# nmonette/TO-UED

Hardware: AMD Instinct MI355X
Metric: agent-env-steps/sec (inner rollout) at num_agents=512; meta-updates/sec (higher is better)
Workload: dtype f32; 1 GPU; C2 LPG meta-gradient env_mode=tabular num_agents=512 num_mini_batches=1 W=64 T=20 K=5 score_function=random; num_agents=512, agents_per_gpu=512, env_workers=64, train_rollout_len=20, num_agent_updates=5, parallelism=dp1 (agent axis)

## Files before the change

to-ued_amd/csrc/gru.hip:

```cpp
#include <stdlib.h>
#include <string.h>
#include <algorithm>
#include "common.h"

extern "C" size_t toued_wgrad_workspace_floats(int ra, int rb, long K);
extern "C" int toued_wgrad(int ra, int rb, long K, const float* A, long lda, const float* B, long ldb, float* C,
                           float* work, size_t work_floats, hipStream_t stream);
extern "C" int toued_wgrad_ldc(int ra, int rb, long K, const float* A, long lda, const float* B, long ldb, float* C,
                               int ldc, float* work, size_t work_floats, hipStream_t stream);
extern "C" size_t toued_rowsum_workspace_floats(int ra, long K);
extern "C" int toued_rowsum_into(int ra, long K, const float* A, long lda, float* C, int ldc, float* work,
                                 size_t work_floats, hipStream_t stream);

typedef float floatx16 __attribute__((ext_vector_type(16)));
typedef float floatx4 __attribute__((ext_vector_type(4)));

#define HU 256
#define RB 32
#define LDH 33
#define NAUG 8
#define KQF 33
#define NTILE_F 32

struct EtaOff {
// ... 748 lines not shown
        const f16x4 h0 = *reinterpret_cast<const f16x4*>(&hB[0][ho]);
        const f16x4 h1 = *reinterpret_cast<const f16x4*>(&hB[1][ho]);
        const bf16x4 hr = *reinterpret_cast<const bf16x4*>(&hB[2][ho]);
        const unsigned sq = quad_soff(cbase + r0, h, g4);
        float sv[3][4];
        float us[3][4];
#pragma unroll
        for (int g = 0; g < 3; ++g) {
          const float4 v = *reinterpret_cast<const float4*>(&usc[g * HU + ub + 8 * g4]);
          us[g][0] = v.x; us[g][1] = v.y; us[g][2] = v.z; us[g][3] = v.w;
        }
        f16x4 n0, n1;
        bf16x4 nr;
#pragma unroll
        for (int e = 0; e < 4; ++e) {
          const int q = 4 * g4 + e;
          const float rg = sigm_r(acc[0][h][q] * us[0][e]);
          const float zg = sigm_r(acc[1][h][q] * us[1][e]);
          const float hn = acc[2][h][q] * us[2][e];
          const float ng = gate_n(ain[h][q], rg, hn);
          const float hin = (((float)h0[e] + (float)h1[e]) + (float)hr[e]) * (1.0f / HSCALE);
          const float hh = (1.0f - zg) * ng + zg * hin;
          split_carry(dn ? 0.0f : hh, n0, n1, nr, e);
          sv[0][e] = rg;
          sv[1][e] = zg;
          sv[2][e] = hn;
          if (SAVE) st_u(rs_hin, vslab, slab_soff(cbase + r0, h, qunit(q)), hin);
          const float rl = fmaxf(hh, 0.0f);
          const float4 w0 = whl[qunit(q) * 3], w1 = whl[qunit(q) * 3 + 1], w2 = whl[qunit(q) * 3 + 2];
          hp_loc[0] += rl * w0.x; hp_loc[1] += rl * w0.y; hp_loc[2] += rl * w0.z;
          hp_loc[3] += rl * w0.w; hp_loc[4] += rl * w1.x; hp_loc[5] += rl * w1.y;
          hp_loc[6] += rl * w1.z; hp_loc[7] += rl * w1.w; hp_loc[8] += rl * w2.x;
        }
        if (SAVE) {
          st4(rs_r, vq, sq, sv[0]);
          st4(rs_z, vq, sq, sv[1]);
          st4(rs_hn, vq, sq, sv[2]);
        }
        *reinterpret_cast<f16x4*>(&hB[0][ho]) = n0;
        *reinterpret_cast<f16x4*>(&hB[1][ho]) = n1;
        *reinterpret_cast<bf16x4*>(&hB[2][ho]) = nr;
      }
#pragma unroll
      for (int oo = 0; oo < 9; ++oo) {
        const float o = __shfl_xor(hp_loc[oo], 32);
        if (hi == 0) hp[(s & 1) * 4608 + (wave * 9 + oo) * 64 + row] = hp_loc[oo] + o;
      }
      GM_STAMP(1 + h);
    }
    FWD_STAMP(3);
    lds_barrier();
    FWD_STAMP(4);
    FWD_STAMP(5);
  }
  if (wave == 0) head_out(T - 1);
}

struct BwdArgs {
  int R, T, W, K;
  const uint8_t* done; long done_stride_k;
  const float4* A;
  const void* A6;
  const float* eta; EtaOff o;
  const float* y_hat; const float* d_pi_hat; const float* d_y_hat;
  const float* s_hin; const float* s_r; const float* s_z; const float* s_n; const float* s_hn;
  long M;
  float* DG;
  float* RH;
  float* DH;
  float* dX3; float* dX4;
  int8_t* CE;
  int F;
  float* SP;
  int stagger, stagger_mode;
  int wg_base;
};
#define SP_C (16 * HU)
#define SP_FLOATS (SP_C + 9 * 64)

template <int NT>
__global__ void __launch_bounds__(512, NT == 1 ? 4 : 1) k_gru_bwd(BwdArgs p) {
  constexpr int RBT = RB * NT;
  constexpr int LDT = RBT + 1;
  __shared__ float dgT[2 * HU * LDT];
  __shared__ float wi34[2 * 3 * HU];
  __shared__ float hv[9 * RBT];
  __shared__ float dxp[NGRP * 2 * RBT];
  const int tid = threadIdx.x, lane = tid & 63, wave = tid >> 6, hi = lane >> 5, col = lane & 31;
  const int nb = p.R / RBT;
  const int k = blockIdx.x / nb;
  const int r0 = (blockIdx.x - k * nb) * RBT;
  const int R = p.R, T = p.T, W = p.W;
  int a_[NT], w_[NT];
#pragma unroll
  for (int h = 0; h < NT; ++h) {
    const int row = r0 + RB * h + col;
    a_[h] = (r0 + RB * h) / W;
    w_[h] = row - a_[h] * W;
  }
  for (int i = tid; i < 2 * 3 * HU; i += 512) {
    const int f = 3 + i / (3 * HU), g = (i / HU) % 3, u = i % HU;
    const int base = g == 0 ? p.o.ir_w : g == 1 ? p.o.iz_w : p.o.in_w;
    wi34[i] = f < p.F ? p.eta[base + f * HU + u] : 0.0f;
  }
  float dh[NT][16];
#pragma unroll
  for (int h = 0; h < NT; ++h)
#pragma unroll
    for (int q = 0; q < 16; ++q) dh[h][q] = 0.0f;
  float wA[5];
#pragma unroll
  for (int kk = 0; kk < 5; ++kk) {
    const int o = 2 * kk + hi, u = 32 * wave + col;
    wA[kk] = o < 9 ? (o == 0 ? p.eta[p.o.pi_w + u] : p.eta[p.o.y_w + u * 8 + (o - 1)]) : 0.0f;
  }
  const uint8_t* done = p.done + (long)k * p.done_stride_k;
  const float4* Ab = p.A + lane;
  const __amdgpu_buffer_rsrc_t rs_hin = rsrc_of(p.s_hin), rs_r = rsrc_of(p.s_r), rs_z = rsrc_of(p.s_z),
                               rs_n = rsrc_of(p.s_n), rs_hn = rsrc_of(p.s_hn), rs_rh = rsrc_of(p.RH);
  const __amdgpu_buffer_rsrc_t rs_dg[4] = {rsrc_of(p.DG), rsrc_of(p.DG + 1L * HU * p.M),
                                           rsrc_of(p.DG + 2L * HU * p.M), rsrc_of(p.DG + 3L * HU * p.M)};
  __syncthreads();
  for (int t = 0; t < T; ++t) {
    const long ctr = ((long)k * T + t) * R;
    if (tid < RBT) {
      const long o = ctr + r0 + tid;
      float yh[8], dy[8], s = 0.0f;
      for (int j = 0; j < 8; ++j) {
        yh[j] = p.y_hat[((long)k * T * 8 + (long)t * 8 + j) * R + r0 + tid];
        dy[j] = p.d_y_hat[((long)k * T * 8 + (long)t * 8 + j) * R + r0 + tid];
        s += yh[j] * dy[j];
      }
      const float dpi = p.d_pi_hat[o];
      hv[tid] = dpi;
      p.DH[o] = dpi;
      for (int j = 0; j < 8; ++j) {
        const float v = yh[j] * (dy[j] - s);
        hv[(j + 1) * RBT + tid] = v;
        p.DH[(long)(j + 1) * p.M + o] = v;
      }
    }
    __syncthreads();
    float dhn_r[NT][16];
    const float* wil = wi34 + 32 * wave + 4 * hi;
#pragma unroll
    for (int h = 0; h < NT; ++h) {
      floatx16 hacc;
#pragma unroll
      for (int q = 0; q < 16; ++q) hacc[q] = 0.0f;
#pragma unroll
      for (int kk = 0; kk < 5; ++kk) {
        const int o = 2 * kk + hi;
        hacc = mfma32(wA[kk], o < 9 ? hv[o * RBT + RB * h + col] : 0.0f, hacc);
      }
      const unsigned vq = (unsigned)((((long)(32 * wave + 4 * hi + (col & 3))) * p.M + r0 + RB * h + (col & 28)) * 4);
      float dx3 = 0.0f, dx4 = 0.0f;
#pragma unroll
      for (int g4 = 0; g4 < 4; ++g4) {
        const unsigned so = (unsigned)(((long)8 * g4 * p.M + ctr) * 4);
        float v_hin[4], v_r[4], v_z[4], v_n[4], v_hn[4];
        ld4(rs_hin, vq, so, v_hin);
        ld4(rs_r, vq, so, v_r);
        ld4(rs_z, vq, so, v_z);
        ld4(rs_n, vq, so, v_n);
        ld4(rs_hn, vq, so, v_hn);
        quad_transpose(v_hin, lane);
        quad_transpose(v_r, lane);
        quad_transpose(v_z, lane);
        quad_transpose(v_n, lane);
        quad_transpose(v_hn, lane);
        float* o_rh = v_hin; float* o_dr = v_r; float* o_dz = v_z; float* o_dhn = v_n; float* o_dn = v_hn;
#pragma unroll
        for (int j = 0; j < 4; ++j) {
          const int q = 4 * g4 + j;
          const float hin = v_hin[j], rg = v_r[j], zg = v_z[j], ng = v_n[j], hn = v_hn[j];
          const float hout = (1.0f - zg) * ng + zg * hin;
          const float d = dh[h][q] + (hout > 0.0f ? hacc[q] : 0.0f);
          const float dn_ = d * (1.0f - zg);
          const float dz = d * (hin - ng);
          const float dnp = dn_ * (1.0f - ng * ng);
          const float dhn = dnp * rg;
          const float drp = dnp * hn * rg * (1.0f - rg);
          const float dzp = dz * zg * (1.0f - zg);
          dh[h][q] = d * zg;
          const int lo = (32 * wave + 4 * hi + qunit(q)) * LDT + RB * h + col;
          dgT[lo] = drp;
          dgT[HU * LDT + lo] = dzp;
          dhn_r[h][q] = dhn;
          o_rh[j] = fmaxf(hout, 0.0f); o_dr[j] = drp; o_dz[j] = dzp; o_dhn[j] = dhn; o_dn[j] = dnp;
          const int qu = qunit(q);
          dx3 += drp * wil[0 * HU + qu] + dzp * wil[1 * HU + qu] + dnp * wil[2 * HU + qu];
          dx4 += drp * wil[3 * HU + qu] + dzp * wil[4 * HU + qu] + dnp * wil[5 * HU + qu];
        }
        {
          const unsigned vb = (unsigned)(((long)(32 * wave + 4 * hi) * p.M + r0 + RB * h + col) * 4);
#pragma unroll
          for (int j = 0; j < 4; ++j) {
            const unsigned so1 = (unsigned)(((long)qunit(4 * g4 + j) * p.M + ctr) * 4);
            st_u(rs_rh, vb, so1, o_rh[j]);
            st_u(rs_dg[3], vb, so1, o_dn[j]);
          }
        }
      }
      dxp[((2 * wave + hi) * 2 + 0) * RBT + RB * h + col] = dx3;
      dxp[((2 * wave + hi) * 2 + 1) * RBT + RB * h + col] = dx4;
    }
    floatx16 acc[NT];
#pragma unroll
    for (int h = 0; h < NT; ++h)
#pragma unroll
      for (int q = 0; q < 16; ++q) acc[h][q] = 0.0f;
#pragma unroll 1
    for (int g = 0; g < 3; ++g) {
      if (g == 2) {
        __syncthreads();
#pragma unroll
        for (int h = 0; h < NT; ++h) {
          float* dgl = dgT + (32 * wave + 4 * hi) * LDT + RB * h + col;
#pragma unroll
          for (int q = 0; q < 16; ++q) dgl[qunit(q) * LDT] = dhn_r[h][q];
        }
      }
      if (g != 1) __syncthreads();
      if (g == 0) {
        store_gate_lds<NT>(dgT, rs_dg[0], p.M, ctr + r0, wave, lane);
        store_gate_lds<NT>(dgT + HU * LDT, rs_dg[1], p.M, ctr + r0, wave, lane);
      } else if (g == 2) {
        store_gate_lds<NT>(dgT, rs_dg[2], p.M, ctr + r0, wave, lane);
      }
      const float* dgs = dgT + (g == 1 ? HU * LDT : 0);
      float4 an = Ab[((wave * 3 + g) * 32 + 0) * 64];
#pragma unroll 2
      for (int kq = 0; kq < 32; ++kq) {
        const float4 av = an;
        if (kq + 1 < 32) an = Ab[((wave * 3 + g) * 32 + kq + 1) * 64];
#pragma unroll
        for (int e = 0; e < 4; ++e) {
          const float x = e == 0 ? av.x : e == 1 ? av.y : e == 2 ? av.z : av.w;
#pragma unroll
          for (int h = 0; h < NT; ++h) {
            const float b = dgs[(2 * (4 * kq + e) + hi) * LDT + RB * h + col];
            acc[h] = mfma32(x, b, acc[h]);
          }
        }
      }
    }
    __syncthreads();
    if (tid < RBT) {
      float s3 = 0.0f, s4 = 0.0f;
      for (int gq = 0; gq < NGRP; ++gq) { s3 += dxp[(gq * 2 + 0) * RBT + tid]; s4 += dxp[(gq * 2 + 1) * RBT + tid]; }
      p.dX3[ctr + r0 + tid] = s3;
      p.dX4[ctr + r0 + tid] = s4;
    }
#pragma unroll
    for (int h = 0; h < NT; ++h) {
      const bool dn = done[((size_t)a_[h] * T + t) * W + w_[h]] != 0;
#pragma unroll
      for (int q = 0; q < 16; ++q) dh[h][q] = dn ? 0.0f : dh[h][q] + acc[h][q];
    }
    __syncthreads();
  }
}


#ifdef BWD_STAMPS
__device__ unsigned long long g_bwd_stamps[64 * 32 * 8];
#define BWD_STAMP(ph)                                                                                  \
  do {                                                                                                 \
    if (blockIdx.x < 64 && tid == 0 && t < 32)                                                         \
      g_bwd_stamps[(blockIdx.x * 32 + t) * 8 + (ph)] = __builtin_amdgcn_s_memtime();                   \
  } while (0)
#define BWD_NWS 8
__device__ unsigned long long g_bwd_wstamps[64 * 32 * 8 * BWD_NWS];
__device__ int g_bwd_wsimd[64 * 8];
#define BWD_WSTAMP(ph)                                                                                 \
  do {                                                                                                 \
    if (blockIdx.x < 64 && lane_now() == 0 && t < 32)                                                  \
      g_bwd_wstamps[((blockIdx.x * 32 + t) * 8 + wave) * BWD_NWS + (ph)] = __builtin_amdgcn_s_memtime(); \
  } while (0)
#else
#define BWD_STAMP(ph) do {} while (0)
#define BWD_WSTAMP(ph) do {} while (0)
#endif

#ifndef BWD_PK
#define BWD_PK 1
#endif
template <bool SMALL>
__global__ void __launch_bounds__(512, 1) k_gru_bwd6n(BwdArgs p) {
  constexpr int RBT = 2 * RB;
  constexpr int PP = HU + 8;
  __shared__ __attribute__((aligned(16))) __bf16 dgB[3][RBT * PP];
  __shared__ float wi34[2 * 3 * HU];
  __shared__ float hv[9 * RBT];
  __shared__ __attribute__((aligned(8))) float dxp[8 * RBT * 2];
  __shared__ __attribute__((aligned(16))) float wsc[HU];
  __shared__ float rmx[8 * RBT];
  __shared__ float wIs[8 * 4 * 64];
  __shared__ float wAs[8 * 5 * 64];
  __shared__ int dns[RBT];
  __shared__ __attribute__((aligned(16))) float Atab[SMALL ? 32 * 64 : 4];
  __shared__ float hvs[SMALL ? 9 * RBT : 1];
  __shared__ floatx4 accl[SMALL ? 8 * 2 * 64 : 1];
  constexpr int DRP = HU + 4;
  static_assert(RBT * DRP * 4 <= 2 * RBT * PP * 2, "dr staging exceeds image slots 1-2");
  float* drs = reinterpret_cast<float*>(&dgB[1][0]);
  const int tid = threadIdx.x, lane = tid & 63, hi = lane >> 5, col = lane & 31;
  const int wave = __builtin_amdgcn_readfirstlane(tid >> 6);
  const int nb = p.R / RBT;
  const int bid = blockIdx.x + p.wg_base;
  const int k = bid / nb;
  const int r0 = (bid - k * nb) * RBT;
  const int R = p.R, T = p.T, W = p.W;
#ifdef BWD_STAMPS
  if (blockIdx.x < 64 && (tid & 63) == 0)
    g_bwd_wsimd[blockIdx.x * 8 + wave] = __builtin_amdgcn_s_getreg((1 << 11) | (4 << 6) | 4);
#endif
  for (int i = tid; i < 2 * 3 * HU; i += 512) {
    const int f = BWD_PK ? 3 + (i & 1) : 3 + i / (3 * HU), g = BWD_PK ? (i >> 1) / HU : (i / HU) % 3,
              u = BWD_PK ? (i >> 1) % HU : i % HU;
    const int base = g == 0 ? p.o.ir_w : g == 1 ? p.o.iz_w : p.o.in_w;
    wi34[i] = f < p.F ? p.eta[base + f * HU + u] : 0.0f;
  }
  for (int i = tid; i < HU; i += 512) wsc[i] = reinterpret_cast<const float*>(p.A6)[B6_SCALES + i];
  const int F = p.F;
  {
    float wI[4];
    load_win_frags(wI, p.eta, p.o, F, wave, lane);
#pragma unroll
    for (int kk = 0; kk < 4; ++kk) wIs[(wave * 4 + kk) * 64 + lane] = wI[kk];
  }
#pragma unroll
  for (int kk = 0; kk < 5; ++kk) {
    const int o = 2 * kk + hi, u = 32 * wave + col;
    wAs[(wave * 5 + kk) * 64 + lane] = o < 9 ? (o == 0 ? p.eta[p.o.pi_w + u] : p.eta[p.o.y_w + u * 8 + (o - 1)]) : 0.0f;
  }
  float dh[2][16];
#pragma unroll
  for (int h = 0; h < 2; ++h)
#pragma unroll
    for (int q = 0; q < 16; ++q) dh[h][q] = 0.0f;
  if (SMALL) {
    for (int i = tid; i < 9 * RBT; i += 512) hvs[i] = 0.0f;
    for (int i = tid; i < 8 * 2 * 64; i += 512) accl[i] = floatx4{0.0f, 0.0f, 0.0f, 0.0f};
  }
  constexpr bool st_rh = !SMALL, st_dn = !SMALL;
  const __amdgpu_buffer_rsrc_t rs_hin = rsrc_of(p.s_hin), rs_r = rsrc_of(p.s_r), rs_z = rsrc_of(p.s_z),
                               rs_hn = rsrc_of(p.s_hn), rs_rh = rsrc_of(SMALL ? p.s_hin : p.RH);
  const __amdgpu_buffer_rsrc_t rs_x = rsrc_of(p.s_hin + (size_t)HU * p.M);
  const __amdgpu_buffer_rsrc_t rs_dg[4] = {rsrc_of(p.DG), rsrc_of(p.DG + 1L * HU * p.M),
                                           rsrc_of(p.DG + 2L * HU * p.M),
                                           rsrc_of(SMALL ? p.DG : p.DG + 3L * HU * p.M)};
  constexpr bool st_DH = !SMALL;
  const __amdgpu_buffer_rsrc_t rs_yh = rsrc_of(p.y_hat), rs_dyh = rsrc_of(p.d_y_hat), rs_dpi = rsrc_of(p.d_pi_hat),
                               rs_DH = rsrc_of(SMALL ? p.dX3 : p.DH), rs_dx3 = rsrc_of(p.dX3), rs_dx4 = rsrc_of(p.dX4),
                               rs_done = rsrc_of(reinterpret_cast<const float*>(p.done + (long)k * p.done_stride_k));
  auto head_cot = [&](int t) {
    if (tid < RBT) {
      const int tl = lane_now();
      const unsigned vrw = (unsigned)tl * 4;
      int dnv;
      {
        const int rw = r0 + tl, a = rw / W;
        dnv = __builtin_amdgcn_raw_buffer_load_b8(rs_done, (a * T + t) * W + rw - a * W, 0, 0);
      }
      const long o = ((long)k * T + t) * R + r0;
      float yh[8], dy[8], s = 0.0f;
#pragma unroll
      for (int j = 0; j < 8; ++j) {
        const unsigned so = (unsigned)((((long)k * T * 8 + (long)t * 8 + j) * R + r0) * 4);
        yh[j] = ld_u(rs_yh, vrw, so);
        dy[j] = ld_u(rs_dyh, vrw, so);
      }
#pragma unroll
      for (int j = 0; j < 8; ++j) s += yh[j] * dy[j];
      const float dpi = ld_u(rs_dpi, vrw, (unsigned)(o * 4));
      float xr[6];
      if (SMALL) {
#pragma unroll
        for (int f = 0; f < 6; ++f)
          xr[f] = ld_u(rs_x, vrw, (unsigned)(((long)(f < F ? f : 0) * p.M + o) * 4));
      }
      dns[tl] = dnv;
      hv[tl] = dpi;
      if (st_DH) st_u(rs_DH, vrw, (unsigned)(o * 4), dpi);
      float hvv[9];
      hvv[0] = dpi;
#pragma unroll
      for (int j = 0; j < 8; ++j) {
        const float v = yh[j] * (dy[j] - s);
        hv[(j + 1) * RBT + tl] = v;
        hvv[j + 1] = v;
        if (st_DH) st_u(rs_DH, vrw, (unsigned)(((long)(j + 1) * p.M + o) * 4), v);
      }
      if (SMALL) {
        float* at = Atab + (tl >> 1) * 64 + 16 * (tl & 1);
#pragma unroll
        for (int c = 0; c < 4; ++c) {
          if (c >= 2) *reinterpret_cast<float4*>(at + 4 * c) = make_float4(0.0f, 0.0f, 0.0f, 0.0f);
          *reinterpret_cast<float4*>(at + 32 + 4 * c) = make_float4(0.0f, 0.0f, 0.0f, 0.0f);
        }
        at[6] = 0.0f;
        at[7] = 0.0f;
        *reinterpret_cast<float4*>(at) = make_float4(0 < F ? xr[0] : 0.0f, 1 < F ? xr[1] : 0.0f, 2 < F ? xr[2] : 0.0f,
                                                     3 < F ? xr[3] : 0.0f);
        *reinterpret_cast<float2*>(at + 4) = make_float2(4 < F ? xr[4] : 0.0f, 5 < F ? xr[5] : 0.0f);
        at[F] = 1.0f;
#pragma unroll
        for (int o9 = 0; o9 < 9; ++o9) at[32 + F + 1 + o9] = hvv[o9];
#pragma unroll
        for (int o9 = 0; o9 < 9; ++o9) hvs[o9 * RBT + tl] += hvv[o9];
      }
    }
  };
  const __amdgpu_buffer_rsrc_t rs_A = rsrc_of(reinterpret_cast<const float*>(p.A6));
  const unsigned vA = (unsigned)lane * 16;
  floatx16 acc[2];
  auto ldAh = [&](int ks, int g, int q) {
    const u32x4 x = __builtin_amdgcn_raw_buffer_load_b128(rs_A, (int)vA,
                                                          (int)((((ks * 8 + wave) * 3 + g) * 3 + q) * 1024), 0);
    return __builtin_bit_cast(f16x8, x);
  };
#ifndef BWD_RD
#define BWD_RD 4
#endif
  auto dg_vbyte = [&](int ub_, int col_) {
    return SMALL ? (unsigned)(ub_ * 128 + col_ * 4) : (unsigned)(((long)ub_ * p.M + r0 + col_) * 4);
  };
  auto dg_soff = [&](long ctr_, int uq, int h) {
    return SMALL ? (unsigned)((((ctr_ + r0) >> 5) + h) * 32768L + uq * 128)
                 : (unsigned)((((long)uq * p.M + ctr_) * 4) + 128 * h);
  };
  auto contract_h = [&](int g) {
    constexpr int RD = BWD_RD;
    f16x8 ring[RD][2], B[2][2];
    int sb = 0, sb1 = 1;
#pragma unroll
    for (int i = 0; i < RD; ++i)
#pragma unroll
      for (int q = 0; q < 2; ++q) ring[i][q] = ldAh(i, g, q);
    const int ln = lane_now(), bl = (ln & 31) * PP + 8 * (ln >> 5);
    auto ldB = [&](int ks, int h) {
#pragma unroll
      for (int q = 0; q < 2; ++q) B[h][q] = *reinterpret_cast<const f16x8*>(&dgB[q ? sb1 : sb][bl + RB * h * PP + 16 * ks]);
    };
    ldB(0, 0);
    ldB(0, 1);
    auto kstep = [&](int ks, f16x8 (&Ar)[2], bool reload) {
#pragma unroll
      for (int h = 0; h < 2; ++h) {
        acc[h] = mfma3h(Ar, B[h], acc[h]);
        if (ks + 1 < 16) ldB(ks + 1, h);
      }
      if (reload) {
#pragma unroll
        for (int q = 0; q < 2; ++q) Ar[q] = ldAh(ks + RD, g, q);
      }
      __builtin_amdgcn_sched_barrier(0);
    };
    constexpr int NG = (16 - RD) / RD;
#pragma nounroll
    for (int gi = 0; gi < NG; ++gi) {
#pragma unroll
      for (int j = 0; j < RD; ++j) kstep(gi * RD + j, ring[j], true);
    }
#pragma unroll
    for (int ks = NG * RD; ks < 16; ++ks) {
      kstep(ks, ring[ks % RD], ks + RD < 16);
      if (ks == 16 - RD) __builtin_amdgcn_sched_barrier(0);
      if (ks >= 12) __builtin_amdgcn_sched_barrier(0);
    }
  };
  auto put4h = [&](int row, int u0, const float (&v)[4], float sc) {
    f16x4 x0, x1;
#pragma unroll
    for (int e = 0; e < 4; ++e) split2h(v[e] * sc, x0, x1, e);
    *reinterpret_cast<f16x4*>(&dgB[0][row * PP + u0]) = x0;
    *reinterpret_cast<f16x4*>(&dgB[1][row * PP + u0]) = x1;
  };
  float* priv = reinterpret_cast<float*>(&dgB[0][0]) + 1056 * wave;
  auto small_mfma = [&](int h, int g4, const float (&dnq)[4], const float (&rhq)[4]) {
    const int ln = lane_now(), row = ln & 31, c = 2 * (g4 & 1) + (ln >> 5);
    const int wo = row * 16 + ((c ^ ((row >> 2) & 3)) << 2);
    *reinterpret_cast<float4*>(priv + wo) = make_float4(dnq[0], dnq[1], dnq[2], dnq[3]);
    *reinterpret_cast<float4*>(priv + 544 + wo) = make_float4(rhq[0], rhq[1], rhq[2], rhq[3]);
    if (g4 & 1) {
      const int l2 = lane_now(), kk = l2 >> 4, j = l2 & 15;
      const int rb = (kk >> 1) * 544 + (kk & 1) * 16 + (j & 3);
      floatx4& al = accl[(wave * 2 + (g4 >> 1)) * 64 + l2];
      floatx4 acc = al;
#pragma unroll
      for (int s2 = 0; s2 < 16; ++s2) {
        const float b = priv[rb + 32 * s2 + ((((j >> 2) ^ ((s2 >> 1) & 3))) << 2)];
        const float a = Atab[(16 * h + s2) * 64 + l2];
        acc = __builtin_amdgcn_mfma_f32_16x16x4f32(a, b, acc, 0, 0, 0);
      }
      al = acc;
    }
  };
#ifndef BWD_NR
#define BWD_NR 3
#endif
  constexpr int NR = BWD_NR;
  const int ub = 32 * wave + 4 * hi;
  float vr[NR][4][4];
  auto load_q = [&](long ctr_, int h, int g4, float (&v)[4][4]) {
    const unsigned vq = quad_vbyte(ub, col), sq = quad_soff(ctr_ + r0, h, g4);
    ld4(rs_hin, slab_vbyte(ub + (col & 3), col & 28), slab_soff(ctr_ + r0, h, 8 * g4), v[0]);
    ld4(rs_r, vq, sq, v[1]);
    ld4(rs_z, vq, sq, v[2]);
    ld4(rs_hn, vq, sq, v[3]);
  };
  float xa[4], xb[4];
  auto load_x = [&](long ctr_, int h, float (&x)[4]) {
#pragma unroll
    for (int kk = 0; kk < 4; ++kk) {
      const int ln = lane_now(), k = 2 * kk + (ln >> 5);
      x[kk] = ld_u(rs_x, (unsigned)((((long)(k < F ? k : 0)) * p.M + RB * h + (ln & 31)) * 4), (unsigned)((ctr_ + r0) * 4));
    }
  };
  auto load_first = [&](long ctr_) {
    load_x(ctr_, 0, xa);
#pragma unroll
    for (int qi = 0; qi < NR - 1; ++qi) load_q(ctr_, qi >> 2, qi & 3, vr[qi]);
  };
  if (p.stagger > 0 && blockIdx.x < 256) {
    const int ph = p.stagger_mode == 0 ? (blockIdx.x >> 3) & 1 : p.stagger_mode == 1 ? blockIdx.x & 1 : (blockIdx.x >> 3) & 3;
    for (int i = 0; i < ph * p.stagger; ++i) __builtin_amdgcn_s_sleep(127);
  }
  const long ctr0 = (long)k * T * R;
  for (int t = 0; t < T; ++t) {
    const long ctr = ctr0 + (long)t * R;
    BWD_STAMP(0);
    head_cot(t);
    lds_barrier();
    BWD_STAMP(1);
    BWD_WSTAMP(0);
    float dz_r[2][16], dhn_r[2][16];
    auto ubn = [&] { return 32 * wave + 4 * (lane_now() >> 5); };
    auto rown = [&](int h) { return RB * h + (lane_now() & 31); };
    auto st_q = [&](__amdgpu_buffer_rsrc_t rs, int h, int g4, const float (&v)[4]) {
#pragma unroll
      for (int e = 0; e < 4; ++e)
        st_u(rs, (unsigned)(((long)ub * p.M + r0 + RB * h + col) * 4),
             (unsigned)(((long)qunit(4 * g4 + e) * p.M + ctr) * 4), v[e]);
    };
    load_first(ctr);
    floatx16 ain;
    floatx16 hacc;
    float dx3 = 0.0f, dx4 = 0.0f;
    float rmr[2] = {0.0f, 0.0f};
#pragma unroll
    for (int qi = 0; qi < 8; ++qi) {
      const int h = qi >> 2, g4 = qi & 3;
      float (&v)[4][4] = vr[qi % NR];
      if (qi + NR - 1 < 8) load_q(ctr, (qi + NR - 1) >> 2, (qi + NR - 1) & 3, vr[(qi + NR - 1) % NR]);
      if (qi == 3) load_x(ctr, 1, xb);
      __builtin_amdgcn_sched_barrier(0);
      if (g4 == 0) {
#pragma unroll
        for (int q = 0; q < 16; ++q) hacc[q] = 0.0f;
#pragma unroll
        for (int kk = 0; kk < 5; ++kk) {
          const int ln = lane_now(), o = 2 * kk + (ln >> 5);
          hacc = mfma32(wAs[(wave * 5 + kk) * 64 + ln], o < 9 ? hv[o * RBT + RB * h + (ln & 31)] : 0.0f, hacc);
        }
        float wI[4];
#pragma unroll
        for (int kk = 0; kk < 4; ++kk) wI[kk] = wIs[(wave * 4 + kk) * 64 + lane];
        ain = gate_ain(wI, F, hi, [&](int k) { return h ? xb[k >> 1] : xa[k >> 1]; });
        dx3 = 0.0f;
        dx4 = 0.0f;
      }
      quad_transpose(v[0], lane);
      const float* wil = wi34 + ubn();
      float drq[4], rhq[4], dnq[4];
      if (BWD_PK) {
        const f2v* wil2 = reinterpret_cast<const f2v*>(wi34) + ubn();
        f2v dx34 = {dx3, dx4};
#pragma unroll
        for (int pp = 0; pp < 2; ++pp) {
          const int j0 = 2 * pp, q0 = 4 * g4 + j0;
          const f2v hin = {v[0][j0], v[0][j0 + 1]}, rg = {v[1][j0], v[1][j0 + 1]}, zg = {v[2][j0], v[2][j0 + 1]},
                    hn = {v[3][j0], v[3][j0 + 1]};
          const f2v ng = {gate_n(ain[q0], rg.x, hn.x), gate_n(ain[q0 + 1], rg.y, hn.y)};
          const f2v omz = 1.0f - zg;
          const f2v hout = omz * ng + zg * hin;
          const f2v hac = {hout.x > 0.0f ? hacc[q0] : 0.0f, hout.y > 0.0f ? hacc[q0 + 1] : 0.0f};
          const f2v d = f2v{dh[h][q0], dh[h][q0 + 1]} + hac;
          const f2v dn_ = d * omz;
          const f2v dz = d * (hin - ng);
          const f2v dnp = dn_ * (1.0f - ng * ng);
          const f2v dhn = dnp * rg;
          const f2v drp = dnp * hn * rg * (1.0f - rg);
          const f2v dzp = dz * zg * omz;
          const f2v dhv = d * zg;
#pragma unroll
          for (int e = 0; e < 2; ++e) {
            const int q = q0 + e, qu = qunit(q);
            dh[h][q] = dhv[e];
            drq[j0 + e] = drp[e];
            dz_r[h][q] = dzp[e];
            dhn_r[h][q] = dhn[e];
            rhq[j0 + e] = fmaxf(hout[e], 0.0f);
            dnq[j0 + e] = dnp[e];
            dx34 += f2v{drp[e], drp[e]} * wil2[0 * HU + qu] + f2v{dzp[e], dzp[e]} * wil2[1 * HU + qu] +
                    f2v{dnp[e], dnp[e]} * wil2[2 * HU + qu];
          }
        }
        dx3 = dx34.x;
        dx4 = dx34.y;
      }
#pragma unroll
      for (int jj = 0; jj < (BWD_PK ? 0 : 4); ++jj) {
        const int q = 4 * g4 + jj;
        const float hin = v[0][jj], rg = v[1][jj], zg = v[2][jj], hn = v[3][jj];
        const float ng = gate_n(ain[q], rg, hn);
        const float hout = (1.0f - zg) * ng + zg * hin;
        const float d = dh[h][q] + (hout > 0.0f ? hacc[q] : 0.0f);
        const float dn_ = d * (1.0f - zg);
        const float dz = d * (hin - ng);
        const float dnp = dn_ * (1.0f - ng * ng);
        const float dhn = dnp * rg;
        const float drp = dnp * hn * rg * (1.0f - rg);
        const float dzp = dz * zg * (1.0f - zg);
        dh[h][q] = d * zg;
        drq[jj] = drp;
        dz_r[h][q] = dzp;
        dhn_r[h][q] = dhn;
        const int qu = qunit(q);
        dx3 += drp * wil[0 * HU + qu] + dzp * wil[1 * HU + qu] + dnp * wil[2 * HU + qu];
        dx4 += drp * wil[3 * HU + qu] + dzp * wil[4 * HU + qu] + dnp * wil[5 * HU + qu];
        rhq[jj] = fmaxf(hout, 0.0f);
        dnq[jj] = dnp;
      }
      if (st_rh) st_q(rs_rh, h, g4, rhq);
      if (st_dn) st_q(rs_dg[3], h, g4, dnq);
      if (SMALL) small_mfma(h, g4, dnq, rhq);
      *reinterpret_cast<float4*>(&drs[rown(h) * DRP + ubn() + 8 * g4]) = make_float4(drq[0], drq[1], drq[2], drq[3]);
#pragma unroll
      for (int jj = 0; jj < 4; ++jj) rmr[h] = fmaxf(rmr[h], fabsf(drq[jj]));
      if (g4 == 3) {
        const float f3 = dx3 + __shfl_xor(dx3, 32), f4 = dx4 + __shfl_xor(dx4, 32);
        const int ln = lane_now();
        if (ln < 32) *reinterpret_cast<float2*>(dxp + (wave * RBT + RB * h + ln) * 2) = make_float2(f3, f4);
      }
      __builtin_amdgcn_sched_barrier(0);
    }
    BWD_STAMP(2);
    BWD_WSTAMP(1);
#pragma unroll
    for (int h = 0; h < 2; ++h) {
      float m = rmr[h];
#pragma unroll
      for (int q = 0; q < 16; ++q) m = fmaxf(m, fmaxf(fabsf(dz_r[h][q]), fabsf(dhn_r[h][q])));
      m = fmaxf(m, __shfl_xor(m, 32));
      const int ln = lane_now();
      if (ln < 32) rmx[wave * RBT + RB * h + ln] = m;
    }
    lds_barrier();
    BWD_STAMP(3);
    float bs[2];
#pragma unroll
    for (int h = 0; h < 2; ++h) {
      float m = 0.0f;
      const int cl = lane_now() & 31;
#pragma unroll
      for (int w8 = 0; w8 < 8; ++w8) m = fmaxf(m, rmx[w8 * RBT + RB * h + cl]);
      int sc = 0, ce = 127;
      if (m > 0.0f && m <= 3.0e38f) {
        int e;
        frexpf(m, &e);
        sc = min(40, max(-40, 14 - e));
        ce = min(126, max(-126, 14 - e));
      }
      bs[h] = ldexpf(1.0f, sc);
      if (p.CE && wave == 0 && lane_now() < 32) p.CE[ctr + r0 + rown(h)] = (int8_t)ce;
    }
    auto store_dg = [&](int g, int row, int g4, const float (&v)[4]) {
#pragma unroll
      for (int e = 0; e < 4; ++e)
        st_u(rs_dg[g], dg_vbyte(ub, col), dg_soff(ctr, qunit(4 * g4 + e), row >= RB ? 1 : 0), v[e]);
    };
    {
      f16x4 x1h[2][4];
#pragma unroll
      for (int h = 0; h < 2; ++h)
#pragma unroll
        for (int g4 = 0; g4 < 4; ++g4) {
          const int row = rown(h), un = ubn();
          const float4 v = *reinterpret_cast<const float4*>(&drs[row * DRP + un + 8 * g4]);
          const float v4[4] = {v.x, v.y, v.z, v.w};
          f16x4 x0;
#pragma unroll
          for (int e = 0; e < 4; ++e) split2h(v4[e] * bs[h], x0, x1h[h][g4], e);
          *reinterpret_cast<f16x4*>(&dgB[0][row * PP + un + 8 * g4]) = x0;
          store_dg(0, RB * h, g4, v4);
        }
      lds_barrier();
#pragma unroll
      for (int h = 0; h < 2; ++h)
#pragma unroll
        for (int g4 = 0; g4 < 4; ++g4)
          *reinterpret_cast<f16x4*>(&dgB[1][rown(h) * PP + ubn() + 8 * g4]) = x1h[h][g4];
      lds_barrier();
    }
    const int un0 = ubn();
#pragma unroll
    for (int g4 = 0; g4 < 4; ++g4) {
      const float4 w4 = *reinterpret_cast<const float4*>(&wsc[un0 + 8 * g4]);
      const float wv[4] = {w4.x, w4.y, w4.z, w4.w};
#pragma unroll
      for (int h = 0; h < 2; ++h)
#pragma unroll
        for (int e = 0; e < 4; ++e) acc[h][4 * g4 + e] = dh[h][4 * g4 + e] * (wv[e] * bs[h]);
    }
    BWD_STAMP(4);
    BWD_WSTAMP(2);
    contract_h(0);
    BWD_WSTAMP(3);
    lds_barrier();
    BWD_WSTAMP(4);
#pragma unroll
    for (int h = 0; h < 2; ++h)
#pragma unroll
      for (int g4 = 0; g4 < 4; ++g4) {
        const float v4[4] = {dz_r[h][4 * g4], dz_r[h][4 * g4 + 1], dz_r[h][4 * g4 + 2], dz_r[h][4 * g4 + 3]};
        put4h(rown(h), ubn() + 8 * g4, v4, bs[h]);
        store_dg(1, RB * h, g4, v4);
      }
    lds_barrier();
    BWD_STAMP(5);
    BWD_WSTAMP(5);
    contract_h(1);
    BWD_WSTAMP(6);
    lds_barrier();
    BWD_WSTAMP(7);
#pragma unroll
    for (int h = 0; h < 2; ++h)
#pragma unroll
      for (int g4 = 0; g4 < 4; ++g4) {
        const float v4[4] = {dhn_r[h][4 * g4], dhn_r[h][4 * g4 + 1], dhn_r[h][4 * g4 + 2], dhn_r[h][4 * g4 + 3]};
        put4h(rown(h), ubn() + 8 * g4, v4, bs[h]);
        store_dg(2, RB * h, g4, v4);
      }
    lds_barrier();
    BWD_STAMP(6);
    contract_h(2);
#pragma unroll
    for (int g4 = 0; g4 < 4; ++g4) {
      const float4 w4 = *reinterpret_cast<const float4*>(&wsc[32 * wave + 4 * (lane_now() >> 5) + 8 * g4]);
      const float wv[4] = {w4.x, w4.y, w4.z, w4.w};
#pragma unroll
      for (int h = 0; h < 2; ++h)
#pragma unroll
        for (int e = 0; e < 4; ++e) acc[h][4 * g4 + e] *= inv_pow2(wv[e] * bs[h]);
    }
    if (tid < RBT) {
      const int tl = lane_now();
      float s3 = 0.0f, s4 = 0.0f;
#pragma unroll
      for (int w8 = 0; w8 < 8; ++w8) {
        const float2 v = *reinterpret_cast<const float2*>(dxp + (w8 * RBT + tl) * 2);
        s3 += v.x;
        s4 += v.y;
      }
      st_u(rs_dx3, (unsigned)tl * 4, (unsigned)((ctr + r0) * 4), s3);
      st_u(rs_dx4, (unsigned)tl * 4, (unsigned)((ctr + r0) * 4), s4);
    }
#pragma unroll
    for (int h = 0; h < 2; ++h) {
      const bool dn = dns[RB * h + (lane_now() & 31)] != 0;
#pragma unroll
      for (int q = 0; q < 16; ++q) dh[h][q] = dn ? 0.0f : acc[h][q];
    }
    BWD_STAMP(7);
    lds_barrier();
  }
  if (SMALL) {
    float* out = p.SP + (size_t)bid * SP_FLOATS;
    const int ln = lane_now();
#pragma unroll
    for (int uh = 0; uh < 2; ++uh) {
      const floatx4 a = accl[(wave * 2 + uh) * 64 + ln];
#pragma unroll
      for (int r = 0; r < 4; ++r) out[(4 * (ln >> 4) + r) * HU + 32 * wave + 16 * uh + (ln & 15)] = a[r];
    }
    for (int i = tid; i < 9 * RBT; i += 512) out[SP_C + i] = hvs[i];
  }
}

__global__ void k_sleep_quanta(int q) {
  for (int i = 0; i < q; ++i) __builtin_amdgcn_s_sleep(127);
}

#define SR_CHUNK 64
__global__ void __launch_bounds__(256) k_small_part(const float* __restrict__ sp, int n_wg, float* __restrict__ part2) {
  const int o = blockIdx.x * 256 + threadIdx.x;
  if (o >= SP_FLOATS) return;
  const int c = blockIdx.y, w0 = c * SR_CHUNK, w1 = min(n_wg, w0 + SR_CHUNK);
  float a = 0.0f;
  for (int w = w0; w < w1; ++w) a += sp[(size_t)w * SP_FLOATS + o];
  part2[(size_t)c * SP_FLOATS + o] = a;
}
__global__ void __launch_bounds__(256) k_small_final(const float* __restrict__ part2, int n_chunk, int F,
                                                     float* __restrict__ GI) {
  const int o = blockIdx.x * 256 + threadIdx.x;
  if (o >= 8 * HU + 9 * (HU + 1)) return;
  float a = 0.0f;
  if (o < 8 * HU) {
    const int i = o / HU, u = o % HU;
    if (i <= F)
      for (int c = 0; c < n_chunk; ++c) a += part2[(size_t)c * SP_FLOATS + i * HU + u];
  } else {
    const int e = o - 8 * HU, oo = e / (HU + 1), u = e % (HU + 1);
    if (u < HU) {
      for (int c = 0; c < n_chunk; ++c) a += part2[(size_t)c * SP_FLOATS + (F + 1 + oo) * HU + u];
    } else {
      for (int c = 0; c < n_chunk; ++c) {
        float rs = 0.0f;
        for (int r = 0; r < 64; ++r) rs += part2[(size_t)c * SP_FLOATS + SP_C + oo * 64 + r];
        a += rs;
      }
    }
  }
  GI[o] = a;
}

}

extern "C" {

int toued_gru_pack(const float* eta, const int* off, int F, float* fwdA, float* bwdA, hipStream_t stream) {
  TOUED_REQUIRE(F >= 1 && F <= 7, "toued_gru_pack: F=%d", F);
  EtaOff o;
  memcpy(&o, off, sizeof(EtaOff));
  const int n1 = NTILE_F * KQF * 64, n2 = 8 * 3 * 32 * 64, n3 = F6_NGRP * 64;
  hipLaunchKernelGGL(k_pack_fwd, dim3((n1 + 255) / 256), dim3(256), 0, stream, eta, o, F,
                     reinterpret_cast<float4*>(fwdA), 0L, 0L);
  hipLaunchKernelGGL(k_fwd6_scales, dim3(16), dim3(256), 0, stream, eta, o, fwdA + (size_t)n1 * 4 + F6_SCALES, 0L, 0L);
  hipLaunchKernelGGL(k_pack_fwd6, dim3((n3 + 255) / 256), dim3(256), 0, stream, eta, o, F,
                     reinterpret_cast<bf16x8*>(fwdA + (size_t)n1 * 4), 0L, 0L);
  hipLaunchKernelGGL(k_pack_bwd, dim3((n2 + 255) / 256), dim3(256), 0, stream, eta, o,
                     reinterpret_cast<float4*>(bwdA));
  hipLaunchKernelGGL(k_bwd6_scales, dim3(HU / 4), dim3(256), 0, stream, eta, o, bwdA + (size_t)n2 * 4 + B6_SCALES);
  hipLaunchKernelGGL(k_pack_bwd6, dim3((16 * 8 * 3 * 64 + 255) / 256), dim3(256), 0, stream, eta, o,
                     reinterpret_cast<__bf16*>(bwdA + (size_t)n2 * 4));
  TOUED_CHECK_LAUNCH();
  return 0;
}

size_t toued_gru_packed_floats(int which) {
  const size_t f32_part = (size_t)NTILE_F * KQF * 64 * 4;
  return which == 1 ? (size_t)8 * 3 * 32 * 64 * 4 + B6_FLOATS : f32_part + F6_FLOATS;
}

static bool gru_f32_forced() {
  static const bool f = [] {
    const char* e = getenv("TOUED_GRU_F32");
    return e && e[0] == '1';
  }();
  return f;
}

static int gru_fwd_launch(int R, int T, int W, int F, const float* X, long xs_f, long xs_col, const uint8_t* done,
                          const float* fwdA, const float* eta, const int* off, float* pi_hat, float* y_hat,
                          float* s_hin, float* s_r, float* s_z, float* s_n, float* s_hn, long M, int save, int rpc,
                          long eta_stride, hipStream_t stream) {
  FwdArgs p;
  p.R = R; p.T = T; p.W = W; p.F = F; p.X = X; p.xs_f = xs_f; p.xs_col = xs_col; p.done = done;
  p.A = reinterpret_cast<const float4*>(fwdA); p.eta = eta;
  p.A6 = fwdA + (size_t)NTILE_F * KQF * 64 * 4;
  memcpy(&p.o, off, sizeof(EtaOff));
  p.pi_hat = pi_hat; p.y_hat = y_hat; p.s_hin = s_hin; p.s_r = s_r; p.s_z = s_z; p.s_n = s_n; p.s_hn = s_hn; p.M = M;
  p.rpc = rpc; p.a_stride4 = (long)toued_gru_packed_floats(2) / 4; p.eta_stride = eta_stride;
  static const int stagger = getenv("TOUED_FWD_STAGGER") ? atoi(getenv("TOUED_FWD_STAGGER")) : 3;
  static const int stagger_save = getenv("TOUED_FWD_STAGGER_SAVE") ? atoi(getenv("TOUED_FWD_STAGGER_SAVE")) : 0;
  p.stagger = save ? stagger_save : stagger;
  const bool nt2 = R % (2 * RB) == 0 && (rpc == 0 || rpc % (2 * RB) == 0);
  if (nt2 && !gru_f32_forced()) {
    if (save) hipLaunchKernelGGL(k_gru_fwd6<true>, dim3(R / (2 * RB)), dim3(512), 0, stream, p);
    else hipLaunchKernelGGL(k_gru_fwd6<false>, dim3(R / (2 * RB)), dim3(512), 0, stream, p);
  } else if (save) {
    if (nt2) hipLaunchKernelGGL((k_gru_fwd<true, 2>), dim3(R / (2 * RB)), dim3(512), 0, stream, p);
    else hipLaunchKernelGGL((k_gru_fwd<true, 1>), dim3(R / RB), dim3(512), 0, stream, p);
  } else {
    if (nt2) hipLaunchKernelGGL((k_gru_fwd<false, 2>), dim3(R / (2 * RB)), dim3(512), 0, stream, p);
    else hipLaunchKernelGGL((k_gru_fwd<false, 1>), dim3(R / RB), dim3(512), 0, stream, p);
  }
  TOUED_CHECK_LAUNCH();
  return 0;
}

int toued_gru_fwd(int R, int T, int W, int F, const float* X, long xs_f, long xs_col, const uint8_t* done,
                  const float* fwdA, const float* eta, const int* off, float* pi_hat, float* y_hat, float* s_hin,
                  float* s_r, float* s_z, float* s_n, float* s_hn, long M, hipStream_t stream) {
  TOUED_REQUIRE(R % RB == 0 && W % RB == 0, "toued_gru_fwd: rows R=%d and workers W=%d must be multiples of 32", R, W);
  TOUED_REQUIRE(F >= 1 && F <= 7 && T >= 1, "toued_gru_fwd: F=%d T=%d", F, T);
  TOUED_REQUIRE((double)M * 264.0 * 4.0 < 4294967295.0, "toued_gru_fwd: M=%ld columns exceed the 4 GiB buffer range "
                "(use --num_mini_batches to split the agent batch)", M);
  TOUED_REQUIRE(s_hin && s_r && s_z && s_n && s_hn, "toued_gru_fwd: saved-activation buffers required");
  return gru_fwd_launch(R, T, W, F, X, xs_f, xs_col, done, fwdA, eta, off, pi_hat, y_hat, s_hin, s_r, s_z, s_n, s_hn,
                        M, 1, 0, 0, stream);
}

int toued_gru_pack_fwd_multi(const float* eta, long eta_stride, int n, const int* off, int F, float* fwdA,
                             hipStream_t stream) {
  TOUED_REQUIRE(F >= 1 && F <= 7 && n >= 0, "toued_gru_pack_fwd_multi: F=%d n=%d", F, n);
  if (n == 0) return 0;
  EtaOff o;
  memcpy(&o, off, sizeof(EtaOff));
  const int n1 = NTILE_F * KQF * 64;
  const long cstride = (long)toued_gru_packed_floats(2);
  hipLaunchKernelGGL(k_pack_fwd, dim3((n1 + 255) / 256, n), dim3(256), 0, stream, eta, o, F,
                     reinterpret_cast<float4*>(fwdA), eta_stride, cstride / 4);
  const int n3 = F6_NGRP * 64;
  hipLaunchKernelGGL(k_fwd6_scales, dim3(16, n), dim3(256), 0, stream, eta, o, fwdA + (size_t)n1 * 4 + F6_SCALES,
                     eta_stride, cstride);
  hipLaunchKernelGGL(k_pack_fwd6, dim3((n3 + 255) / 256, n), dim3(256), 0, stream, eta, o, F,
                     reinterpret_cast<bf16x8*>(fwdA + (size_t)n1 * 4), eta_stride, cstride / 4);
  TOUED_CHECK_LAUNCH();
  return 0;
}

int toued_gru_fwd_multi(int R, int T, int W, int F, int rows_per_cand, const float* X, long xs_f, long xs_col,
                        const uint8_t* done, const float* fwdA, const float* eta, long eta_stride, const int* off,
                        float* pi_hat, float* y_hat, hipStream_t stream) {
  TOUED_REQUIRE(R % RB == 0 && W % RB == 0, "toued_gru_fwd_multi: rows R=%d and workers W=%d must be multiples of 32",
                R, W);
  TOUED_REQUIRE(rows_per_cand > 0 && rows_per_cand % RB == 0 && R % rows_per_cand == 0,
                "toued_gru_fwd_multi: rows_per_cand=%d must be a multiple of 32 dividing R=%d", rows_per_cand, R);
  TOUED_REQUIRE(F >= 1 && F <= 7 && T >= 1, "toued_gru_fwd_multi: F=%d T=%d", F, T);
  return gru_fwd_launch(R, T, W, F, X, xs_f, xs_col, done, fwdA, eta, off, pi_hat, y_hat, nullptr, nullptr, nullptr,
                        nullptr, nullptr, 0, 0, rows_per_cand, eta_stride, stream);
}

int toued_gru_bwd_col_exp(int R) { return R % (2 * RB) == 0 && !gru_f32_forced() ? 1 : 0; }

int toued_gru_bwd(int R, int T, int W, int K, const uint8_t* done, long done_stride_k, const float* bwdA,
                  const float* eta, const int* off, const float* y_hat, const float* d_pi_hat, const float* d_y_hat,
                  const float* s_hin, const float* s_r, const float* s_z, const float* s_n, const float* s_hn, long M,
                  float* DG, float* RH, float* DH, float* dX3, float* dX4, int8_t* col_exp, hipStream_t stream) {
  TOUED_REQUIRE(R % RB == 0 && W % RB == 0, "toued_gru_bwd: rows R=%d and workers W=%d must be multiples of 32", R, W);
  TOUED_REQUIRE((double)M * 264.0 * 4.0 < 4294967295.0, "toued_gru_bwd: M=%ld columns exceed the 4 GiB buffer range",
                M);
  BwdArgs p{};
  p.R = R; p.T = T; p.W = W; p.K = K; p.done = done; p.done_stride_k = done_stride_k;
  p.A = reinterpret_cast<const float4*>(bwdA); p.eta = eta;
  p.A6 = bwdA + (size_t)8 * 3 * 32 * 64 * 4;
  memcpy(&p.o, off, sizeof(EtaOff));
  p.y_hat = y_hat; p.d_pi_hat = d_pi_hat; p.d_y_hat = d_y_hat;
  p.s_hin = s_hin; p.s_r = s_r; p.s_z = s_z; p.s_n = s_n; p.s_hn = s_hn; p.M = M;
  p.DG = DG; p.RH = RH; p.DH = DH; p.dX3 = dX3; p.dX4 = dX4; p.CE = col_exp;
  p.F = (p.o.ir_b - p.o.in_w) / HU;
  TOUED_REQUIRE(p.F >= 1 && p.F <= 7 && p.o.ir_b - p.o.in_w == p.F * HU, "toued_gru_bwd: LPG layout F=%d", p.F);
  p.SP = nullptr;
  if (toued_gru_bwd_col_exp(R))
    hipLaunchKernelGGL(k_gru_bwd6n<false>, dim3(K * (R / (2 * RB))), dim3(512), 0, stream, p);
  else
    hipLaunchKernelGGL(k_gru_bwd<1>, dim3(K * (R / RB)), dim3(512), 0, stream, p);
  TOUED_CHECK_LAUNCH();
  return 0;
}

int toued_gru_slab_saves(int R) { return toued_gru_bwd_col_exp(R); }

int toued_gru_bwd_fused_fits(int R, int F) { return toued_gru_bwd_col_exp(R) && F >= 1 && F <= 6 ? 1 : 0; }

size_t toued_gru_bwd_fused_work_floats(int R, int K) {
  const long n_wg = (long)K * (R / (2 * RB)), n_chunk = (n_wg + SR_CHUNK - 1) / SR_CHUNK;
  return (size_t)(n_wg + n_chunk) * SP_FLOATS;
}

int toued_gru_bwd_fused(int R, int T, int W, int K, const uint8_t* done, long done_stride_k, const float* bwdA,
                        const float* eta, const int* off, const float* y_hat, const float* d_pi_hat,
                        const float* d_y_hat, const float* s_hin, const float* s_r, const float* s_z,
                        const float* s_hn, long M, float* DG3, float* dX3, float* dX4, int8_t* col_exp, float* GI,
                        float* work, size_t work_floats, hipStream_t stream) {
  TOUED_REQUIRE(R % (2 * RB) == 0 && W % RB == 0 && !gru_f32_forced(),
                "toued_gru_bwd_fused: rows R=%d must be a multiple of 64 (W=%d), split-precision kernels", R, W);
  TOUED_REQUIRE((double)M * 264.0 * 4.0 < 4294967295.0, "toued_gru_bwd_fused: M=%ld columns exceed the 4 GiB range",
                M);
  TOUED_REQUIRE(M == (long)K * T * R, "toued_gru_bwd_fused: M=%ld != K*T*R", M);
  TOUED_REQUIRE(work_floats >= toued_gru_bwd_fused_work_floats(R, K), "toued_gru_bwd_fused: workspace %zu < %zu",
                work_floats, toued_gru_bwd_fused_work_floats(R, K));
  TOUED_REQUIRE(col_exp != nullptr, "toued_gru_bwd_fused: col_exp is required");
  BwdArgs p{};
  p.R = R; p.T = T; p.W = W; p.K = K; p.done = done; p.done_stride_k = done_stride_k;
  p.A = reinterpret_cast<const float4*>(bwdA); p.eta = eta;
  p.A6 = bwdA + (size_t)8 * 3 * 32 * 64 * 4;
  memcpy(&p.o, off, sizeof(EtaOff));
  p.y_hat = y_hat; p.d_pi_hat = d_pi_hat; p.d_y_hat = d_y_hat;
  p.s_hin = s_hin; p.s_r = s_r; p.s_z = s_z; p.s_n = nullptr; p.s_hn = s_hn; p.M = M;
  p.DG = DG3; p.RH = nullptr; p.DH = nullptr; p.dX3 = dX3; p.dX4 = dX4; p.CE = col_exp;
  p.F = (p.o.ir_b - p.o.in_w) / HU;
  TOUED_REQUIRE(p.F >= 1 && p.F <= 6 && p.o.ir_b - p.o.in_w == p.F * HU, "toued_gru_bwd_fused: LPG layout F=%d", p.F);
  const int n_wg = K * (R / (2 * RB)), n_chunk = (n_wg + SR_CHUNK - 1) / SR_CHUNK;
  p.SP = work;
  {
    static const char* e = getenv("TOUED_BWD_STAGGER");
    p.stagger = e ? atoi(e) : 0;
    p.stagger_mode = e && strchr(e, ',') ? atoi(strchr(e, ',') + 1) : 0;
  }
  float* part2 = work + (size_t)n_wg * SP_FLOATS;
  static const int halves = getenv("TOUED_BWD_HALVES") ? atoi(getenv("TOUED_BWD_HALVES")) : -1;
  if (halves >= 0 && n_wg >= 2) {
    static hipStream_t sh[2] = {nullptr, nullptr};
    static hipEvent_t ev[3];
    if (!sh[0]) {
      int dev = 0, ncu = 0;
      TOUED_REQUIRE(hipGetDevice(&dev) == hipSuccess &&
                        hipDeviceGetAttribute(&ncu, hipDeviceAttributeMultiprocessorCount, dev) == hipSuccess,
                    "toued_gru_bwd_fused: device query failed");
      uint32_t m[2][16] = {};
      for (int c = 0; c < ncu && c < 512; ++c) m[c & 1][c >> 5] |= 1u << (c & 31);
      const uint32_t nw = (uint32_t)((ncu + 31) / 32);
      for (int h = 0; h < 2; ++h)
        TOUED_REQUIRE(hipExtStreamCreateWithCUMask(&sh[h], nw, m[h]) == hipSuccess, "CU-masked stream");
      for (int i = 0; i < 3; ++i) TOUED_REQUIRE(hipEventCreateWithFlags(&ev[i], hipEventDisableTiming) == hipSuccess, "ev");
    }
    (void)hipEventRecord(ev[0], stream);
    const int n1 = n_wg / 2;
    for (int h = 0; h < 2; ++h) {
// ... 63 lines not shown
```

Before: 180.9 million agent-env-steps/sec.

## Prefetch first GRU backward quad tile into LDS via buffer-load DMA

Replaces the row-major dr staging layout with per-wave/per-lane cells, which frees space in the LDS image slots. It then issues buffer_load...lds DMA for the first quad (hin, r, z, hn) of the next timestep, overlapping it with the current step's contraction. The first quad is read from LDS instead of global memory. The cost is added vmcnt waits and inline assembly that manipulates m0, plus a risk of LDS aliasing between the dr cells and the DMA target slot.

```diff
diff --git a/to-ued_amd/csrc/gru.hip b/to-ued_amd/csrc/gru.hip
--- a/to-ued_amd/csrc/gru.hip
+++ b/to-ued_amd/csrc/gru.hip
@@ -1074,16 +1074,49 @@
   __shared__ __attribute__((aligned(16))) float Atab[SMALL ? 32 * 64 : 4];
   __shared__ float hvs[SMALL ? 9 * RBT : 1];
   __shared__ floatx4 accl[SMALL ? 8 * 2 * 64 : 1];
-  constexpr int DRP = HU + 4;
-  static_assert(RBT * DRP * 4 <= 2 * RBT * PP * 2, "dr staging exceeds image slots 1-2");
+  constexpr int DRC = 8 * 64 * 4;
+  static_assert(4 * DRC * 4 <= RBT * PP * 2, "four qi of dr staging cells exceed one image slot");
   float* drs = reinterpret_cast<float*>(&dgB[1][0]);
+  constexpr int DRS2 = RBT * PP / 2;
   const int tid = threadIdx.x, lane = tid & 63, hi = lane >> 5, col = lane & 31;
   const int wave = __builtin_amdgcn_readfirstlane(tid >> 6);
+  auto drcell = [&](int qi) { return drs + (qi >> 2) * DRS2 + ((qi & 3) * 8 + wave) * 256 + lane_now() * 4; };
   const int nb = p.R / RBT;
   const int bid = blockIdx.x + p.wg_base;
   const int k = bid / nb;
   const int r0 = (bid - k * nb) * RBT;
   const int R = p.R, T = p.T, W = p.W;
+  const __amdgpu_buffer_rsrc_t rs_hin = rsrc_of(p.s_hin), rs_r = rsrc_of(p.s_r), rs_z = rsrc_of(p.s_z),
+                               rs_hn = rsrc_of(p.s_hn);
+  const unsigned pf_lds = (unsigned)(uintptr_t)(&dgB[2][0]) + 1024u * (unsigned)wave;
+  auto prefetch_q0 = [&](long ctr_) {
+    const int ln = lane_now(), cl = ln & 31, ubl = 32 * wave + 4 * (ln >> 5);
+    const unsigned vs = slab_vbyte(ubl + (cl & 3), cl & 28), vq = quad_vbyte(ubl, cl);
+    const unsigned so = __builtin_amdgcn_readfirstlane(quad_soff(ctr_ + r0, 0, 0));
+    const unsigned dst = __builtin_amdgcn_readfirstlane(pf_lds);
+    unsigned keep;
+    static_assert(GRU_LD_AUX == 2, "the DMA below carries the loads' nt bit");
+    asm volatile(
+        "s_waitcnt lgkmcnt(0)\n\t"
+        "s_mov_b32 %0, m0\n\t"
+        "s_mov_b32 m0, %8\n\t"
+        "s_nop 4\n\t"
+        "buffer_load_dwordx4 %1, %3, %7 offen nt lds\n\t"
+        "s_add_u32 m0, m0, 0x2000\n\t"
+        "s_nop 0\n\t"
+        "buffer_load_dwordx4 %2, %4, %7 offen nt lds\n\t"
+        "s_add_u32 m0, m0, 0x2000\n\t"
+        "s_nop 0\n\t"
+        "buffer_load_dwordx4 %2, %5, %7 offen nt lds\n\t"
+        "s_add_u32 m0, m0, 0x2000\n\t"
+        "s_nop 0\n\t"
+        "buffer_load_dwordx4 %2, %6, %7 offen nt lds\n\t"
+        "s_mov_b32 m0, %0"
+        : "=&s"(keep)
+        : "v"(vs), "v"(vq), "s"(rs_hin), "s"(rs_r), "s"(rs_z), "s"(rs_hn), "s"(so), "s"(dst)
+        : "memory", "scc");
+  };
+  if (T > 0) prefetch_q0((long)k * T * R);
 #ifdef BWD_STAMPS
   if (blockIdx.x < 64 && (tid & 63) == 0)
     g_bwd_wsimd[blockIdx.x * 8 + wave] = __builtin_amdgcn_s_getreg((1 << 11) | (4 << 6) | 4);
@@ -1117,8 +1150,7 @@
     for (int i = tid; i < 8 * 2 * 64; i += 512) accl[i] = floatx4{0.0f, 0.0f, 0.0f, 0.0f};
   }
   constexpr bool st_rh = !SMALL, st_dn = !SMALL;
-  const __amdgpu_buffer_rsrc_t rs_hin = rsrc_of(p.s_hin), rs_r = rsrc_of(p.s_r), rs_z = rsrc_of(p.s_z),
-                               rs_hn = rsrc_of(p.s_hn), rs_rh = rsrc_of(SMALL ? p.s_hin : p.RH);
+  const __amdgpu_buffer_rsrc_t rs_rh = rsrc_of(SMALL ? p.s_hin : p.RH);
   const __amdgpu_buffer_rsrc_t rs_x = rsrc_of(p.s_hin + (size_t)HU * p.M);
   const __amdgpu_buffer_rsrc_t rs_dg[4] = {rsrc_of(p.DG), rsrc_of(p.DG + 1L * HU * p.M),
                                            rsrc_of(p.DG + 2L * HU * p.M),
@@ -1294,13 +1326,19 @@
   auto load_first = [&](long ctr_) {
     load_x(ctr_, 0, xa);
 #pragma unroll
-    for (int qi = 0; qi < NR - 1; ++qi) load_q(ctr_, qi >> 2, qi & 3, vr[qi]);
+    for (int qi = 1; qi < NR - 1; ++qi) load_q(ctr_, qi >> 2, qi & 3, vr[qi]);
+#pragma unroll
+    for (int a = 0; a < 4; ++a) {
+      const float4 v = *reinterpret_cast<const float4*>(drcell(4 + a));
+      vr[0][a][0] = v.x; vr[0][a][1] = v.y; vr[0][a][2] = v.z; vr[0][a][3] = v.w;
+    }
   };
   if (p.stagger > 0 && blockIdx.x < 256) {
     const int ph = p.stagger_mode == 0 ? (blockIdx.x >> 3) & 1 : p.stagger_mode == 1 ? blockIdx.x & 1 : (blockIdx.x >> 3) & 3;
     for (int i = 0; i < ph * p.stagger; ++i) __builtin_amdgcn_s_sleep(127);
   }
   const long ctr0 = (long)k * T * R;
+  asm volatile("s_waitcnt vmcnt(0)" ::: "memory");
   for (int t = 0; t < T; ++t) {
     const long ctr = ctr0 + (long)t * R;
     BWD_STAMP(0);
@@ -1409,7 +1447,7 @@
       if (st_rh) st_q(rs_rh, h, g4, rhq);
       if (st_dn) st_q(rs_dg[3], h, g4, dnq);
       if (SMALL) small_mfma(h, g4, dnq, rhq);
-      *reinterpret_cast<float4*>(&drs[rown(h) * DRP + ubn() + 8 * g4]) = make_float4(drq[0], drq[1], drq[2], drq[3]);
+      *reinterpret_cast<float4*>(drcell(qi)) = make_float4(drq[0], drq[1], drq[2], drq[3]);
 #pragma unroll
       for (int jj = 0; jj < 4; ++jj) rmr[h] = fmaxf(rmr[h], fabsf(drq[jj]));
       if (g4 == 3) {
@@ -1461,7 +1499,7 @@
 #pragma unroll
         for (int g4 = 0; g4 < 4; ++g4) {
           const int row = rown(h), un = ubn();
-          const float4 v = *reinterpret_cast<const float4*>(&drs[row * DRP + un + 8 * g4]);
+          const float4 v = *reinterpret_cast<const float4*>(drcell(4 * h + g4));
           const float v4[4] = {v.x, v.y, v.z, v.w};
           f16x4 x0;
 #pragma unroll
@@ -1469,6 +1507,7 @@
           *reinterpret_cast<f16x4*>(&dgB[0][row * PP + un + 8 * g4]) = x0;
           store_dg(0, RB * h, g4, v4);
         }
+      if (t + 1 < T) prefetch_q0(ctr + R);
       lds_barrier();
 #pragma unroll
       for (int h = 0; h < 2; ++h)
@@ -1491,6 +1530,7 @@
     BWD_WSTAMP(2);
     contract_h(0);
     BWD_WSTAMP(3);
+    asm volatile("s_waitcnt vmcnt(0)" ::: "memory");
     lds_barrier();
     BWD_WSTAMP(4);
 #pragma unroll
```

New measurement: 181.4 million agent-env-steps/sec (median of 6 runs). No clear change (+0.3%).
